# goroda/GPEXP

Hardware: AMD Instinct MI355X
Metric: GP-fit+IVAR-eval points/s at N=32768 d=8 (wall-time in ms_per_step); value = (N+M)/t_step, SURVEY 8d's N/t_fit and M/t_IVAR are points_per_s_fit / points_per_s_ivar right behind it (higher is better)
Workload: dtype f64; 1 GPU; C4: N=32768 d=8 Matern-5/2 (rho=0.5,s=1,noise=0.1) kfill+potrf+potrs+logdet+IVAR over M=32768 MC points; N=32768, d=8, M=32768, kernel=matern52, seed=32768, parallelism=1 GPU

## Files before the change

gpexp_amd/_lib.py:

```python
import ctypes as C
import os

import numpy as np

_HERE = os.path.dirname(os.path.abspath(__file__))
LIB_PATH = os.path.join(_HERE, "libgpx_hip.so")

c_i64 = C.c_int64
c_dp = C.POINTER(C.c_double)
c_ip = C.POINTER(c_i64)
c_vp = C.c_void_p

_SIGS = {
    "gpx_abi_version": (C.c_int, []),
    "gpx_last_error": (C.c_char_p, []),
    "gpx_create": (C.c_int, [C.c_int, C.POINTER(c_vp)]),
    "gpx_destroy": (C.c_int, [c_vp]),
    "gpx_sync": (C.c_int, [c_vp]),
    "gpx_trim": (C.c_int, [c_vp]),
    "gpx_device_info": (C.c_int, [c_vp, C.c_char_p, C.c_int, C.POINTER(C.c_int), c_ip, C.POINTER(C.c_int)]),
    "gpx_mat_from_host": (C.c_int, [c_vp, c_dp, c_i64, c_i64, C.c_int, C.POINTER(c_vp)]),
    "gpx_mat_alloc": (C.c_int, [c_vp, c_i64, c_i64, C.c_int, C.POINTER(c_vp)]),
    "gpx_mat_free": (C.c_int, [c_vp, c_vp]),
    "gpx_mat_clone": (C.c_int, [c_vp, c_vp, C.POINTER(c_vp)]),
# ... 149 lines not shown
    "gpx_program_capture": (C.c_int, [c_vp, c_ip, c_i64, c_ip, c_i64, C.POINTER(c_vp)]),
    "gpx_graph_launch": (C.c_int, [c_vp, c_vp, c_dp, c_ip]),
    "gpx_graph_free": (C.c_int, [c_vp, c_vp]),
    "gpx_dist2_unpack_rows": (C.c_int, [c_vp, c_vp, c_i64, c_i64, c_i64, c_i64, c_vp, c_i64, c_i64, c_i64]),
    "gpx_dist2_unpack_diag": (C.c_int, [c_vp, c_vp, c_i64, c_i64, c_i64, c_vp, c_i64]),
    "gpx_dist2_unpack_diag_at": (C.c_int, [c_vp, c_vp, c_i64, c_i64, c_i64, c_vp, c_i64, c_i64]),
    "gpx_dist2_trsv_diag": (C.c_int, [c_vp, c_vp, c_i64, c_i64, c_i64, c_vp, c_i64, C.c_int]),
    "gpx_dist2_gemv": (C.c_int, [c_vp, c_vp, c_i64, c_i64, c_i64, c_i64, c_vp, c_i64, c_vp, c_i64, C.c_int]),
    "gpx_dist2_logdet_acc": (C.c_int, [c_vp, c_vp, c_i64, c_i64, c_i64, c_i64, c_vp]),
    "gpx_stream_select": (C.c_int, [c_vp, C.c_int]),
    "gpx_event_record": (C.c_int, [c_vp, C.c_int]),
    "gpx_event_wait": (C.c_int, [c_vp, C.c_int]),
    "gpx_dist_finish": (C.c_int, [c_vp, c_vp]),
    "gpx_ivar_grad": (C.c_int, [c_vp, C.c_int, C.c_int, c_dp, C.c_int, c_vp, c_vp, c_vp, c_dp, c_dp]),
    "gpx_ivar_grad_w": (C.c_int, [c_vp, C.c_int, C.c_int, c_dp, C.c_int, c_vp, c_vp, c_vp, c_dp, c_vp, c_dp]),
    "gpx_ivar_grad_rows": (C.c_int, [c_vp, C.c_int, C.c_int, c_dp, C.c_int, c_vp, c_vp, c_vp, c_vp, c_i64, c_dp]),
    "gpx_var_grad": (C.c_int, [c_vp, C.c_int, C.c_int, c_dp, C.c_int, c_vp, c_vp, c_vp, c_dp, c_dp, c_dp, c_dp]),
    "gpx_var_grad_newpt": (C.c_int, [c_vp, C.c_int, C.c_int, c_dp, C.c_int, c_vp, c_vp, c_vp, c_dp]),
    "gpx_fitc_var_grad": (C.c_int, [c_vp, c_vp, C.c_int, C.c_int, c_dp, C.c_int, c_vp, c_vp, c_dp, c_dp, c_dp, c_dp]),
    "gpx_fitc_var_grad_newpt": (C.c_int, [c_vp, c_vp, C.c_int, C.c_int, c_dp, C.c_int, c_vp, c_vp, c_dp]),
    "gpx_vfe_design_create": (C.c_int, [c_vp, C.c_int, C.c_int, c_dp, C.c_int, c_vp, C.c_double, c_vp, C.POINTER(c_vp)]),
    "gpx_vfe_design_pin": (C.c_int, [c_vp, c_vp, c_vp]),
    "gpx_vfe_design_eval": (C.c_int, [c_vp, c_vp, c_vp, c_dp, c_dp]),
    "gpx_vfe_design_shape": (C.c_int, [c_vp, C.POINTER(c_i64), C.POINTER(c_i64), C.POINTER(c_i64)]),
    "gpx_vfe_design_free": (C.c_int, [c_vp, c_vp]),
    "gpx_vfe_var_grad": (C.c_int, [c_vp, c_vp, C.c_int, C.c_int, c_dp, C.c_int, c_vp, c_vp, c_vp, c_dp]),
    "gpx_vfe_var_grad_newpt": (C.c_int, [c_vp, c_vp, c_vp, c_vp, c_dp]),
    "gpx_profile_enable": (C.c_int, [c_vp, C.c_int]),
    "gpx_profile_reset": (C.c_int, [c_vp]),
    "gpx_profile_get": (C.c_int, [c_vp, C.c_int, c_ip, c_dp, c_dp, c_dp]),
    "gpx_dbg_gemm": (C.c_int, [c_vp, c_vp, c_vp, c_vp, C.c_int, C.c_int, C.c_int]),
    "gpx_dbg_gemm_strassen": (C.c_int, [c_vp, c_vp, c_vp, c_vp]),
    "gpx_dbg_gemm_strassen_depth": (C.c_int, [c_vp, c_vp, c_vp, c_vp, C.c_int]),
    "gpx_dbg_gemm_tri": (C.c_int, [c_vp, c_vp, c_vp, c_vp, C.c_int, C.c_int, C.c_int]),
    "gpx_dbg_gemm_ksplit": (C.c_int, [c_vp, c_vp, c_vp, c_vp, C.c_int, C.c_int]),
    "gpx_dbg_kfill_plan": (C.c_int, [c_vp, C.c_int, C.c_int, c_dp, C.c_int, c_vp, c_vp, C.POINTER(C.c_int), c_dp]),
    "gpx_dbg_colreduce_plan": (C.c_int, [c_i64, c_i64, C.POINTER(c_i64), C.POINTER(c_i64)]),
    "gpx_dbg_colreduce": (C.c_int, [c_vp, c_vp, c_i64, c_dp, c_dp, C.c_int]),
    "gpx_dbg_rowreduce": (C.c_int, [c_vp, c_vp, c_i64, c_dp, C.c_int, c_dp]),
    "gpx_dbg_sum": (C.c_int, [c_vp, c_dp, c_i64, c_dp]),
    "gpx_dbg_panel_bcast_plan": (C.c_int, [C.c_int, C.c_int, c_i64, C.c_int, C.POINTER(c_i64), C.POINTER(C.c_int),
                                           C.POINTER(c_i64), c_i64, C.POINTER(c_i64)]),
    "gpx_dbg_guard_violations": (c_i64, [c_vp]),
    "gpx_dbg_guard_selftest": (C.c_int, [c_vp]),
    "gpx_dbg_pool_stats": (C.c_int, [c_vp, C.POINTER(c_i64), C.POINTER(c_i64)]),
    "gpx_dbg_spin": (C.c_int, [c_vp, C.c_int]),
    "gpx_dbg_spin_us": (C.c_int, [c_vp, c_i64]),
    "gpx_dbg_stamp": (C.c_int, [c_vp, C.c_int]),
    "gpx_dbg_spin_until": (C.c_int, [c_vp, C.c_int, c_i64]),
    "gpx_dbg_event_elapsed": (C.c_int, [c_vp, C.c_int, C.c_int, c_dp]),
    "gpx_dbg_leaf_stamps": (C.c_int, [c_vp, c_vp, C.c_int, C.POINTER(c_i64)]),
    "gpx_dbg_greedy_var_scores": (C.c_int, [c_vp, C.c_int, C.c_int, c_dp, C.c_int, c_vp, c_ip, c_i64, c_dp]),
    "gpx_dbg_acq_epilogue": (C.c_int, [c_vp, C.c_int, C.c_double, c_dp, c_dp, c_i64, c_i64, c_dp, c_dp, C.POINTER(c_i64),
                                       c_dp]),
    "gpx_dbg_acq_mes_epilogue": (C.c_int, [c_vp, c_dp, c_i64, C.c_int, c_dp, c_dp, c_i64, c_i64, c_dp, c_dp, C.POINTER(c_i64), c_dp]),
}

_lib = None


def load():
    global _lib
    if _lib is not None:
        return _lib
    path = os.environ.get("GPX_LIB_PATH", LIB_PATH)
    if not os.path.exists(path):
# ... 49 lines not shown
```

gpexp_amd/csrc/api.hip:

```cpp
#include "gpx_internal.h"
#include <stdarg.h>
#include <stdio.h>
#include <string.h>
#include <math.h>
#include <stdlib.h>

static thread_local char g_err[1024] = "";

void gpx_set_error(const char* fmt, ...) {
  va_list ap;
  va_start(ap, fmt);
  vsnprintf(g_err, sizeof(g_err), fmt, ap);
  va_end(ap);
}

static constexpr int64_t GUARD = 4096;

int gpx_dev_alloc(gpx_ctx* ctx, int64_t bytes, void** out) {
  if (bytes <= 0) bytes = 8;
  bytes = gpx_round_up(bytes, 256);
  const int64_t key = bytes + (ctx->guard ? 2 * GUARD : 0);
  void* base = nullptr;
  auto it = ctx->pool.find(key);
  if (it != ctx->pool.end()) {
// ... 1318 lines not shown
                   : launch_gemm_ksplit_small(ctx, A->p, A->ld, B->p, B->ld, C->p, C->ld, m, n, k, mode == 3, parts, P);
}

int gpx_dbg_gemm(gpx_ctx* ctx, const gpx_mat* A, const gpx_mat* B, gpx_mat* C, int bt, int accumulate, int lower) {
  GPX_ARG(ctx && A && B && C, "NULL argument");
  const int64_t m = C->prows, n = C->pcols, k = A->pcols;
  GPX_ARG(A->prows == m, "A rows");
  GPX_ARG(bt ? (B->prows == n && B->pcols == k) : (B->prows == k && B->pcols == n), "B shape");
  GPX_TRY(launch_gemm(ctx, A->p, A->ld, B->p, B->ld, C->p, C->ld, m, n, k, bt != 0, accumulate != 0,
                      lower != 0));
  GPX_HIP(hipStreamSynchronize(ctx->stream));
  return 0;
}

int gpx_dbg_gemm_strassen(gpx_ctx* ctx, const gpx_mat* A, const gpx_mat* B, gpx_mat* C) {
  GPX_ARG(ctx && A && B && C, "NULL argument");
  const int64_t m = C->prows, n = C->pcols, k = A->pcols;
  GPX_ARG(A->prows == m && B->prows == k && B->pcols == n, "operand shapes");
  GPX_TRY(launch_gemm_strassen(ctx, A->p, A->ld, B->p, B->ld, C->p, C->ld, m, n, k, 1, nullptr, 0));
  GPX_HIP(hipStreamSynchronize(ctx->stream));
  return 0;
}

int gpx_dbg_gemm_strassen_depth(gpx_ctx* ctx, const gpx_mat* A, const gpx_mat* B, gpx_mat* C, int depth) {
  GPX_ARG(ctx && A && B && C, "NULL argument");
  GPX_ARG(depth >= 0 && depth <= GPX_STRASSEN_MAX_DEPTH, "strassen: depth out of range");
  const int64_t m = C->prows, n = C->pcols, k = A->pcols;
  GPX_ARG(A->prows == m && B->prows == k && B->pcols == n, "operand shapes");
  GPX_TRY(launch_gemm_strassen(ctx, A->p, A->ld, B->p, B->ld, C->p, C->ld, m, n, k, depth, nullptr, 0));
  GPX_HIP(hipStreamSynchronize(ctx->stream));
  return 0;
}

}
```

gpexp_amd/csrc/chol.hip:

```cpp
#include "gpx_internal.h"
#include <algorithm>
#include <math.h>
#include <stdlib.h>
#include <stddef.h>

namespace {

constexpr int NB = GPX_TILE;
constexpr int LS = NB + 1;

typedef double d4 __attribute__((ext_vector_type(4)));

__device__ __forceinline__ double readlane_d(double v, int srclane) {
  int lo = __builtin_amdgcn_readlane(__double2loint(v), srclane);
  int hi = __builtin_amdgcn_readlane(__double2hiint(v), srclane);
  return __hiloint2double(hi, lo);
}

constexpr int LB = 16;
constexpr int TS17 = LB + 1;
constexpr int BSZ = LB * TS17;
constexpr int LEAF_CB = LB * LB + 64 + LB;

__device__ __forceinline__ constexpr int sb_off(int I, int J) { return (I * (I + 1) / 2 + J) * BSZ; }
// ... 1208 lines not shown
    const int64_t o = blk_off(P, b0), sz = blk_off(P, b0 + 1) - o;
    hipLaunchKernelGGL(binv_gemv_kernel, dim3((unsigned)((sz + 3) / 4)), dim3(256), 0, ctx->stream, blk_inv(P, P.binvT, b0),
                       P.sib, sz, rhs + o, z + o, 0);
    return 0;
  }
  const int64_t mid = (b0 + b1) / 2;
  GPX_TRY(potrs_bwd(ctx, P, mid, b1, rhs, z));
  const int64_t r0 = blk_off(P, mid), r1 = blk_off(P, b1), c0 = blk_off(P, b0);
  GPX_TRY(launch_colreduce(ctx, P.L + r0 * P.ld + c0, P.ld, r1 - r0, r0 - c0, z + r0, rhs + c0, P.part, 1));
  return potrs_bwd(ctx, P, b0, mid, rhs, z);
}

#ifndef GPX_STRASSEN_MIN_ROWS
#define GPX_STRASSEN_MIN_ROWS 8192
#endif
#ifndef GPX_STRASSEN_MIN_COLS
#define GPX_STRASSEN_MIN_COLS 4096
#endif
#ifndef GPX_STRASSEN2_MIN_ROWS
#define GPX_STRASSEN2_MIN_ROWS 16384
#endif
#ifndef GPX_STRASSEN2_MIN_COLS
#define GPX_STRASSEN2_MIN_COLS 16384
#endif
static inline int strassen_gate(int64_t rows, int64_t cols, int64_t k) {
  if (!(rows >= GPX_STRASSEN_MIN_ROWS && k >= GPX_STRASSEN_MIN_ROWS && cols >= GPX_STRASSEN_MIN_COLS &&
        gemm_strassen_scratch_bytes(rows, cols, k, 1) > 0))
    return 0;
  if (!(rows >= GPX_STRASSEN2_MIN_ROWS && k >= GPX_STRASSEN2_MIN_ROWS && cols >= GPX_STRASSEN2_MIN_COLS &&
        gemm_strassen_scratch_bytes(rows, cols, k, 2) > 0))
    return 1;
  return 2;
}

static int trsm_left_oop_rec(gpx_ctx* ctx, const PotrsPlan& P, int64_t b0, int64_t b1, double* B, int64_t ldb, double* W,
                             int64_t ldw, int64_t m) {
  if (b1 - b0 == 1) {
    const int64_t o = blk_off(P, b0), sz = blk_off(P, b0 + 1) - o;
    return launch_gemm_tri(ctx, blk_inv(P, P.binv, b0), P.sib, B + o * ldb, ldb, W + o * ldw, ldw, sz, m, sz, false, false,
                           false, 1);
  }
  const int64_t mid = (b0 + b1) / 2;
  GPX_TRY(trsm_left_oop_rec(ctx, P, b0, mid, B, ldb, W, ldw, m));
  const int64_t r0 = blk_off(P, mid), r1 = blk_off(P, b1), c0 = blk_off(P, b0);
  const int depth = P.strassen ? std::min(P.strassen, strassen_gate(r1 - r0, m, r0 - c0)) : 0;
  if (depth > 0)
    GPX_TRY(launch_gemm_strassen(ctx, P.L + r0 * P.ld + c0, P.ld, W + c0 * ldw, ldw, B + r0 * ldb, ldb, r1 - r0, m, r0 - c0,
                                 depth, P.sscr, P.sscr_bytes));
  else
    GPX_TRY(launch_gemm(ctx, P.L + r0 * P.ld + c0, P.ld, W + c0 * ldw, ldw, B + r0 * ldb, ldb, r1 - r0, m, r0 - c0, false,
                        true, false));
  return trsm_left_oop_rec(ctx, P, mid, b1, B, ldb, W, ldw, m);
}

int chol_trsm_left_oop(gpx_ctx* ctx, gpx_mat* Lm, double* B, int64_t ldb, double* W, int64_t ldw, int64_t m) {
  GPX_ARG(Lm && Lm->factored && Lm->aux && B && W && B != W, "trsm: matrix has not been factored / bad buffers");
  if (m == 0) return 0;
  GPX_TRY(chol_binv_ensure(ctx, Lm));
  PotrsPlan P;
  P.L = Lm->p;
  P.ld = Lm->ld;
  P.n = Lm->prows;
  P.sib = Lm->binv_ib;
  P.ib = P.sib < 1024 ? P.sib : 1024;
  P.nblk = (P.n + P.ib - 1) / P.ib;
  P.binv = Lm->binv;
  P.binvT = nullptr;
  P.part = nullptr;
  void* ps = nullptr;
  int64_t sbytes = 0;
  int depth = 0;
  const int64_t max_depth = env_i64("GPX_STRASSEN", GPX_STRASSEN_MAX_DEPTH);
  if (P.nblk >= 2 && max_depth > 0) {
    const int64_t r0 = blk_off(P, P.nblk / 2);
    for (depth = (int)std::min<int64_t>(max_depth, strassen_gate(P.n - r0, m, r0)); depth > 0; --depth) {
      sbytes = gemm_strassen_scratch_bytes(P.n - r0, m, r0, depth);
      if (sbytes > 0 && gpx_dev_alloc(ctx, sbytes, &ps) == 0) break;
      (void)hipGetLastError();
// ... 105 lines not shown
```

gpexp_amd/csrc/gemm_f64.hip:

```cpp
#include "gpx_internal.h"
#include <stdlib.h>

namespace {

typedef double d4 __attribute__((ext_vector_type(4)));

constexpr int KB = 16;
constexpr int SA = KB + 1;

template <bool BT, int TE>
struct Smem {
  double a[2][TE * SA];
  double b[2][BT ? TE * SA : KB * (TE + 16)];
};

template <bool LOWER>
__device__ __forceinline__ bool tile_of(int sblk, int within, int tiles_m, int tiles_n, int sb_cols, int sb_shift,
                                        int* by, int* bx, int rot = 0) {
  const int sbm = (1 << sb_shift) - 1;
  int sr, sc;
  if (LOWER) {
    const int nsr = (tiles_m + sbm) >> sb_shift;
    const int noff = nsr * (nsr - 1) / 2;
    if (sblk < noff) {
// ... 397 lines not shown
  gemm_tile<false, true, TE, NoSeg, Multi>(sm, A, lda, B, ldb, dst.c[0], ldc, nk, by, bx, NoSeg(), dst);
}

template <bool BSIDE>
__global__ __launch_bounds__(256) void strassen_sums_kernel(const double* __restrict__ X, int64_t ldx, int64_t hr, int64_t hc,
                                                            double* __restrict__ S, int64_t lds, int64_t sstride) {
  const int64_t j = ((int64_t)blockIdx.x * 256 + threadIdx.x) * 2;
  if (j >= hc) return;
  for (int64_t i = blockIdx.y; i < hr; i += gridDim.y) {
    const double* x1 = X + i * ldx + j;
    const double* x2 = X + (i + hr) * ldx + j;
    const double2 x11 = *reinterpret_cast<const double2*>(x1);
    const double2 x12 = *reinterpret_cast<const double2*>(x1 + hc);
    const double2 x21 = *reinterpret_cast<const double2*>(x2);
    const double2 x22 = *reinterpret_cast<const double2*>(x2 + hc);
    double* o = S + i * lds + j;
#define GPX_S2(k_, ex_, ey_) *reinterpret_cast<double2*>(o + (k_) * sstride) = make_double2(ex_, ey_)
    GPX_S2(0, x11.x + x22.x, x11.y + x22.y);
    if (BSIDE) {
      GPX_S2(1, x12.x - x22.x, x12.y - x22.y);
      GPX_S2(2, x21.x - x11.x, x21.y - x11.y);
      GPX_S2(3, x11.x + x12.x, x11.y + x12.y);
      GPX_S2(4, x21.x + x22.x, x21.y + x22.y);
    } else {
      GPX_S2(1, x21.x + x22.x, x21.y + x22.y);
      GPX_S2(2, x11.x + x12.x, x11.y + x12.y);
      GPX_S2(3, x21.x - x11.x, x21.y - x11.y);
      GPX_S2(4, x12.x - x22.x, x12.y - x22.y);
    }
#undef GPX_S2
  }
}

template <bool BT, bool ACC>
__global__ __launch_bounds__(256, 2) void gemm_f64_batched_kernel(const double* A, int64_t lda, int64_t sa,
                                                                  const double* B, int64_t ldb, int64_t sb, double* C,
                                                                  int64_t ldc, int64_t sc, int nk, int tiles_n, int hiprio) {
  __shared__ Smem<BT, 64> sm;
  if (hiprio) __builtin_amdgcn_s_setprio(3);
  const int64_t b = blockIdx.y;
  const int by = blockIdx.x / tiles_n, bx = blockIdx.x - by * tiles_n;
  gemm_tile<BT, ACC, 64>(sm, A + b * sa, lda, B + b * sb, ldb, C + b * sc, ldc, nk, by, bx);
}

template <bool LOWER>
__global__ __launch_bounds__(256, 2) void gemm_f64_ksplit_kernel(const double* A, int64_t lda, const double* B, int64_t ldb,
                                                                 double* P, int64_t n, int64_t sp, int nk_slice, int parts,
                                                                 int tiles_m, int tiles_n, int sb_cols, int sb_shift) {
  __shared__ Smem<true, 128> sm;
  const int w = blockIdx.x, xcd = w & 7, q = w >> 3, sbs2 = 2 * sb_shift;
  const int job = (q >> sbs2) * 8 + xcd, within = q & ((1 << sbs2) - 1);
  int sb, slice;
  if (LOWER) {
    const int nsr = (tiles_m + (1 << sb_shift) - 1) >> sb_shift, noff = nsr * (nsr - 1) / 2;
    if (job < parts * noff) {
      slice = job / noff;
      sb = job - slice * noff;
    } else {
      const int jj = job - parts * noff;
      slice = jj / nsr;
      sb = noff + jj - slice * nsr;
    }
  } else {
    const int nsb = ((tiles_m + (1 << sb_shift) - 1) >> sb_shift) * sb_cols;
    slice = job / nsb;
    sb = job - slice * nsb;
// ... 278 lines not shown
  GPX_ARG(m % 128 == 0 && n % 128 == 0 && k % KB == 0 && k > 0 && m > 0 && n > 0, "gemm: m,n must be multiples of 128 and k of 16");
  GPX_ARG((lda % 2) == 0 && (ldb % 2) == 0, "gemm: leading dimensions must be even (16-byte loads)");
  GPX_ARG(dst.nd >= 1 && dst.nd <= GPX_MULTI_MAX, "gemm: bad destination count");
  const double tiles128 = (double)(m / 128) * (double)(n / 128);
  const int te = tiles128 < 1024.0 ? 64 : 128;
  const Plan p = make_plan(m, n, false, te);
  GPX_ARG(p.wgs < ((int64_t)1 << 31), "gemm: grid too large");
  const int nk = (int)(k / KB);
  ProfScope ps(ctx, GPX_PROF_GEMM, 2.0 * (double)m * (double)n * (double)k, 0.0);
  if (te == 64)
    hipLaunchKernelGGL(gemm_f64_multi_kernel<64>, dim3((unsigned)p.wgs), dim3(256), 0, ctx->stream, A, lda, B, ldb, dst, ldc, nk,
                       p.tm, p.tn, p.sbc, p.sb_shift);
  else
    hipLaunchKernelGGL(gemm_f64_multi_kernel<128>, dim3((unsigned)p.wgs), dim3(256), 0, ctx->stream, A, lda, B, ldb, dst, ldc, nk,
                       p.tm, p.tn, p.sbc, p.sb_shift);
  GPX_HIP(hipGetLastError());
  return 0;
}

static inline bool strassen_shape_ok(int64_t m, int64_t n, int64_t k, int depth) {
  return depth >= 1 && depth <= GPX_STRASSEN_MAX_DEPTH && m > 0 && n > 0 && k > 0 && m % ((int64_t)128 << depth) == 0 &&
         n % ((int64_t)128 << depth) == 0 && k % ((int64_t)KB << depth) == 0;
}

static inline int64_t strassen_level_elems(int64_t hm, int64_t hn, int64_t hk) {
  return 5 * (hm * gpx_skew_ld(hk) + hk * gpx_skew_ld(hn));
}

int64_t gemm_strassen_scratch_bytes(int64_t m, int64_t n, int64_t k, int depth) {
  if (!strassen_shape_ok(m, n, k, depth)) return 0;
  int64_t elems = 0;
  for (int d = 0; d < depth; ++d) {
    m /= 2, n /= 2, k /= 2;
    elems += strassen_level_elems(m, n, k);
  }
  return elems * 8;
}

namespace {
struct SDest {
  double* c;
  double s;
};
struct SProd {
  int a, b, nq, q[2];
  double s[2];
};
constexpr SProd kStrassen[7] = {
    {-1, -1, 2, {0, 3}, {1.0, 1.0}},
    {-2, 0, 2, {2, 3}, {1.0, -1.0}},
    {0, -2, 2, {1, 3}, {1.0, 1.0}},
    {3, -3, 2, {0, 2}, {1.0, 1.0}},
    {-3, 3, 2, {1, 0}, {1.0, -1.0}},
    {-4, -4, 1, {3, 0}, {1.0, 0.0}},
    {-5, -5, 1, {0, 0}, {1.0, 0.0}},
};
}

static int strassen_rec(gpx_ctx* ctx, const double* A, int64_t lda, const double* B, int64_t ldb, const SDest* dst, int nd,
                        int64_t ldc, int64_t m, int64_t n, int64_t k, int depth, double* scratch) {
  if (depth == 0) {
    for (int d = 1; d < nd; ++d)
      for (int e = 0; e < d; ++e) GPX_ARG(dst[d].c != dst[e].c, "strassen: two destinations of one product coincide");
    if (nd == 1 && dst[0].s == 1.0) return launch_gemm(ctx, A, lda, B, ldb, dst[0].c, ldc, m, n, k, false, true, false);
    if (nd == 2 && dst[0].s == 1.0) return launch_gemm_dual(ctx, A, lda, B, ldb, dst[0].c, dst[1].c, dst[1].s, ldc, m, n, k);
    GPX_ARG(nd >= 1 && nd <= GPX_MULTI_MAX, "strassen: too many destinations for one product");
    Multi md;
    for (int d = 0; d < GPX_MULTI_MAX; ++d) {
      md.c[d] = d < nd ? dst[d].c : nullptr;
      md.s[d] = d < nd ? dst[d].s : 0.0;
    }
    md.nd = nd;
    return launch_gemm_multi(ctx, A, lda, B, ldb, md, ldc, m, n, k);
  }
  const int64_t hm = m / 2, hn = n / 2, hk = k / 2, lsa = gpx_skew_ld(hk), lsb = gpx_skew_ld(hn);
  const int64_t sa = hm * lsa, sb = hk * lsb;
  double* const S = scratch;
  double* const T = scratch + 5 * sa;
  double* const below = T + 5 * sb;
  {
    ProfScope ps(ctx, GPX_PROF_REDUCE, 5.0 * (double)hm * hk + 5.0 * (double)hk * hn, 72.0 * ((double)hm * hk + (double)hk * hn));
    hipLaunchKernelGGL(strassen_sums_kernel<false>, dim3((unsigned)((hk / 2 + 255) / 256), (unsigned)(hm < 65535 ? hm : 65535)),
                       dim3(256), 0, ctx->stream, A, lda, hm, hk, S, lsa, sa);
    hipLaunchKernelGGL(strassen_sums_kernel<true>, dim3((unsigned)((hn / 2 + 255) / 256), (unsigned)(hk < 65535 ? hk : 65535)),
                       dim3(256), 0, ctx->stream, B, ldb, hk, hn, T, lsb, sb);
    if (hipGetLastError() != hipSuccess) {
      gpx_set_error("strassen: operand-sum launch failed");
      return -2;
    }
  }
  const int64_t qoff[4] = {0, hn, hm * ldc, hm * ldc + hn};
  for (const SProd& p : kStrassen) {
    const double* Ap = p.a < 0 ? S + (-1 - p.a) * sa : (p.a == 0 ? A : A + hm * lda + hk);
    const double* Bp = p.b < 0 ? T + (-1 - p.b) * sb : (p.b == 0 ? B : B + hk * ldb + hn);
    SDest sub[GPX_MULTI_MAX];
    int ns = 0;
    for (int d = 0; d < nd; ++d)
      for (int j = 0; j < p.nq; ++j) {
        GPX_ARG(ns < GPX_MULTI_MAX, "strassen: too many destinations for one product");
        sub[ns++] = SDest{dst[d].c + qoff[p.q[j]], dst[d].s * p.s[j]};
      }
    GPX_TRY(strassen_rec(ctx, Ap, p.a < 0 ? lsa : lda, Bp, p.b < 0 ? lsb : ldb, sub, ns, ldc, hm, hn, hk, depth - 1, below));
  }
  return 0;
}

int launch_gemm_strassen(gpx_ctx* ctx, const double* A, int64_t lda, const double* B, int64_t ldb, double* C, int64_t ldc,
                         int64_t m, int64_t n, int64_t k, int depth, double* scratch, int64_t scratch_bytes) {
  if (depth > GPX_STRASSEN_MAX_DEPTH) depth = GPX_STRASSEN_MAX_DEPTH;
  if ((lda % 2) != 0 || (ldb % 2) != 0 || C == A || C == B) depth = 0;
  void* own = nullptr;
  int64_t need = 0;
  for (; depth > 0; --depth) {
    need = gemm_strassen_scratch_bytes(m, n, k, depth);
    if (need == 0) continue;
    if (scratch && scratch_bytes >= need) break;
    if (gpx_dev_alloc(ctx, need, &own) == 0) {
      scratch = (double*)own;
      break;
    }
    (void)hipGetLastError();
    own = nullptr;
  }
  if (depth <= 0) return launch_gemm(ctx, A, lda, B, ldb, C, ldc, m, n, k, false, true, false);
  const SDest top{C, 1.0};
  const int r = strassen_rec(ctx, A, lda, B, ldb, &top, 1, ldc, m, n, k, depth, scratch);
  if (own) {
    (void)hipStreamSynchronize(ctx->stream);
    gpx_dev_release(ctx, own, need);
  }
  return r;
}

int launch_dist2_update(gpx_ctx* ctx, double* C, int64_t ldc, int64_t lr0, int64_t m, int64_t lc0, int64_t n, int64_t nb, int Pr,
                        int Pc, int pr, int pc, int64_t piece_stride, int64_t dsz, int nseg, const double* const* g,
                        const int64_t* ks, int below_diag) {
  if (m == 0 || n == 0 || nseg == 0) return 0;
  GPX_ARG(nseg > 0 && nseg <= GPX_SEG_MAX && Pr >= 1 && Pr <= GPX_MAX_PR && Pc >= 1, "dist2 update: too many segments / grid rows");
  GPX_ARG(m % 128 == 0 && n % 128 == 0 && nb % 128 == 0 && lr0 % nb == 0 && lc0 % nb == 0 && (ldc % 2) == 0, "dist2 update: alignment");
  Dist2Upd u;
  for (int s = 0; s < nseg; ++s) {
    u.g[s] = g[s];
    for (int p = 0; p < Pr; ++p) u.li0[s][p] = (int)(ks[s] + 1 <= p ? 0 : (ks[s] - p) / Pr + 1);
  }
  u.nseg = nseg;
  u.seg_nk = (int)(nb / KB);
  u.Pr = Pr; u.Pc = Pc; u.pr = pr; u.pc = pc;
  u.nb = (int)nb;
  u.gld = (int)gpx_g_ld(nb);
  u.li_first = (int)(lr0 / nb);
  u.lj_first = (int)(lc0 / nb);
  u.below_diag = below_diag;
  u.piece_stride = piece_stride;
  u.dsz = dsz;
  double tiles128 = 0.0;
  for (int64_t lj = lc0 / nb; lj * nb < lc0 + n; ++lj) {
    const int64_t J = lj * Pc + pc;
    const int64_t cw = (lc0 + n - lj * nb) < nb ? (lc0 + n - lj * nb) : nb;
    for (int64_t li = lr0 / nb; li * nb < lr0 + m; ++li) {
// ... 56 lines not shown
```

gpexp_amd/csrc/gpx_internal.h:

```cpp
#pragma once
#include <hip/hip_runtime.h>
#include <stdint.h>
#include <stdlib.h>
#include <string>
#include <vector>
#include <map>
#include <memory>
#include <unordered_set>
#include "../../include/gpx.h"
#include "../../include/gpx_dist.h"
#include "../../include/gpx_debug.h"

#define GPX_TILE 128
#define GPX_MAXD GPX_MAX_DIM
#define GPX_NSTREAMS 6
#define GPX_SEG_MAX 8
#ifndef GPX_G_SKEW
#define GPX_G_SKEW 0
#endif
#define GPX_MAX_PR 4

void gpx_set_error(const char* fmt, ...);
#define GPX_HIP(call)                                                                   \
  do {                                                                                  \
// ... 239 lines not shown
int gpx_posterior_chunk(gpx_ctx* ctx, const KParams& kp, const gpx_mat* L, const gpx_mat* X, const double* Zc, int64_t mc,
                        double* B, double* Wout, const double* alpha_dev, double* mean_dev, double* mean_host, double* ssq,
                        double* kd, double* part);
int posterior_cov_into(gpx_ctx* ctx, const KParams& kp, const gpx_mat* L, const gpx_mat* X, const gpx_mat* Z, Scratch& sc, double* C,
                       int64_t ldc);
int gpx_model_or_prior(const gpx_mat* L, const gpx_mat* X, const double* alpha, const char* msg, bool* prior);

int launch_kfill(gpx_ctx* ctx, const KParams& kp, const double* A, int64_t na, const double* B, int64_t nb,
                 int symmetric, const double* d_nugget, int64_t nugget_len, double nugget_scalar,
                 double* out, int64_t prows, int64_t pcols, int64_t ld);
int launch_kfill_offset(gpx_ctx* ctx, const KParams& kp, const double* X, int64_t n, int64_t row_off, int64_t col_off,
                        const double* d_nugget, int64_t nugget_len, double nugget_scalar, double* out, int64_t prows,
                        int64_t pcols, int64_t ld);
int launch_kdiag(gpx_ctx* ctx, const KParams& kp, const double* Z, int64_t m, double* out);
int launch_kfill_cyclic(gpx_ctx* ctx, const KParams& kp, const double* X, int64_t n, const double* d_nugget,
                        int64_t nugget_len, double nugget_scalar, double* out, int64_t prows, int64_t pcols, int64_t ld,
                        int64_t nb, int Pr, int pr, int Pc, int pc);
int gpx_copy2d(gpx_ctx* ctx, const double* src, int64_t lds_, double* dst, int64_t ldd, int64_t rows, int64_t cols);
int gpx_copy2d_lower(gpx_ctx* ctx, const double* src, int64_t lds_, double* dst, int64_t ldd, int64_t n);
int launch_kfill_rows(gpx_ctx* ctx, const KParams& kp, const double* X, int64_t n, int64_t row0, const double* d_nugget,
                      int64_t nugget_len, double nugget_scalar, double* out, int64_t prows_band, int64_t pcols,
                      int64_t ld);

static inline int gpx_chain_prio(const gpx_ctx* ctx) { return ctx->stream == ctx->streams[1] ? 1 : 0; }
int launch_gemm(gpx_ctx* ctx, const double* A, int64_t lda, const double* B, int64_t ldb, double* C, int64_t ldc,
                int64_t m, int64_t n, int64_t k, bool bt, bool accumulate, bool lower);

int launch_gemm_tri(gpx_ctx* ctx, const double* A, int64_t lda, const double* B, int64_t ldb, double* C, int64_t ldc,
                    int64_t m, int64_t n, int64_t k, bool bt, bool accumulate, bool lower, int tri);
constexpr int GPX_STRASSEN_MAX_DEPTH = 2;
int64_t gemm_strassen_scratch_bytes(int64_t m, int64_t n, int64_t k, int depth);
int launch_gemm_strassen(gpx_ctx* ctx, const double* A, int64_t lda, const double* B, int64_t ldb, double* C, int64_t ldc,
                         int64_t m, int64_t n, int64_t k, int depth, double* scratch, int64_t scratch_bytes);
int launch_gemm_ksplit(gpx_ctx* ctx, const double* A, int64_t lda, const double* B, int64_t ldb, double* C, int64_t ldc,
                       int64_t m, int64_t n, int64_t k, bool lower, int64_t parts, double* P, bool assign = false);
int launch_gemm_ksplit_small(gpx_ctx* ctx, const double* A, int64_t lda, const double* B, int64_t ldb, double* C, int64_t ldc,
                             int64_t m, int64_t n, int64_t k, bool assign, int64_t parts, double* P);
int launch_gemm_batched(gpx_ctx* ctx, const double* A, int64_t lda, int64_t sa, const double* B, int64_t ldb, int64_t sb,
                        double* C, int64_t ldc, int64_t sc, int64_t m, int64_t n, int64_t k, bool bt, bool accumulate,
                        int64_t batch);

int launch_dist2_update(gpx_ctx* ctx, double* C, int64_t ldc, int64_t lr0, int64_t m, int64_t lc0, int64_t n, int64_t nb, int Pr,
                        int Pc, int pr, int pc, int64_t piece_stride, int64_t dsz, int nseg, const double* const* g,
                        const int64_t* ks, int below_diag);

int launch_leaf(gpx_ctx* ctx, double* A, int64_t ld, double* inv, int64_t base_index, int64_t n_valid);
int chol_potrf(gpx_ctx* ctx, double* A, int64_t ld, int64_t n, double* invd, int64_t n_valid);
int chol_potrf_nozero(gpx_ctx* ctx, double* A, int64_t ld, int64_t n, double* invd, int64_t base, int64_t n_valid);
int chol_trsm_right(gpx_ctx* ctx, const double* L, int64_t ldl, const double* invd, double* X, int64_t ldx,
                    int64_t m, int64_t n);
int chol_trsm_right_n(gpx_ctx* ctx, const double* L, int64_t ldl, const double* invd, double* X, int64_t ldx,
                      int64_t m, int64_t n);
int chol_trsm_left(gpx_ctx* ctx, const double* L, int64_t ldl, const double* invd, double* B, int64_t ldb,
                   int64_t n, int64_t m);
int chol_trsv(gpx_ctx* ctx, const double* L, int64_t ld, const double* invd, double* y, int64_t n, bool transposed);
int64_t chol_trsv_scratch_bytes(int64_t n);
int chol_trsv_with_scratch(gpx_ctx* ctx, const double* L, int64_t ld, const double* invd, double* y, int64_t n,
                           bool transposed, double* scratch);
int launch_logdet(gpx_ctx* ctx, const double* L, int64_t ld, int64_t n, double* d_out);
int chol_trtri(gpx_ctx* ctx, const gpx_mat* L, double* Linv, double* tmp);
int chol_binv_ensure(gpx_ctx* ctx, gpx_mat* L);
int chol_trsm_right_trailing(gpx_ctx* ctx, gpx_mat* L, int64_t r0, double* X, int64_t ldx, int64_t m, int transposed, double* T);
int chol_trsm_right_leading(gpx_ctx* ctx, gpx_mat* L, int64_t ncols, double* X, int64_t ldx, int64_t m, double* T, int64_t tcap);
int chol_trsm_right_n_leading(gpx_ctx* ctx, gpx_mat* L, int64_t ncols, double* X, int64_t ldx, int64_t m, double* T);
int chol_block_inverse(gpx_ctx* ctx, const double* D, int64_t ldd, const double* invd, double* inv, int64_t w, double* tmp);
int64_t chol_binv_order(int64_t n);
// ... 137 lines not shown
```

gpexp_amd/device.py:

```python
import ctypes as C
import atexit
import os

import numpy as np

from . import _lib
from ._lib import check, as_f64, dptr, c_vp, c_i64, GpxError

K_SE, K_MATERN32, K_MATERN52, K_MEHLER = 0, 1, 2, 3
PROF_CLASSES = ["kfill", "gemm", "leaf", "trsv", "reduce", "greedy", "comm", "kcross"]

_ctx = None


class Context:

    def __init__(self, device=None):
        self.lib = _lib.load()
        if device is None:
            device = int(os.environ.get("LOCAL_RANK", "0"))
        h = c_vp()
        rc = self.lib.gpx_create(int(device), C.byref(h))
        if rc != 0:
            raise RuntimeError("gpexp_amd needs an MI355X: " + self.lib.gpx_last_error().decode())
# ... 1135 lines not shown


def var_grad_newpt(ctx, spec, L, X, Z):
    out = np.empty(Z.shape[0] * spec.d)
    check(ctx.lib.gpx_var_grad_newpt(ctx.h, *spec.args(), L.h, X.h, Z.h, dptr(out)))
    return out


def kfill_plan(ctx, spec, X, Z=None):
    ex = C.c_int()
    cen = np.zeros(spec.d)
    check(ctx.lib.gpx_dbg_kfill_plan(ctx.h, *spec.args(), X.h, Z.h if Z is not None else None, C.byref(ex), dptr(cen)))
    return bool(ex.value), cen


def dbg_gemm_tri(ctx, A, B, Cm, bt, accumulate, tri):
    check(ctx.lib.gpx_dbg_gemm_tri(ctx.h, A.h, B.h, Cm.h, int(bt), int(accumulate), int(tri)))


def dbg_gemm_ksplit(ctx, A, B, Cm, mode, parts):
    check(ctx.lib.gpx_dbg_gemm_ksplit(ctx.h, A.h, B.h, Cm.h, int(mode), int(parts)))


def dbg_gemm(ctx, A, B, Cm, bt, accumulate, lower=False):
    check(ctx.lib.gpx_dbg_gemm(ctx.h, A.h, B.h, Cm.h, int(bt), int(accumulate), int(lower)))


def dbg_gemm_strassen(ctx, A, B, Cm):
    check(ctx.lib.gpx_dbg_gemm_strassen(ctx.h, A.h, B.h, Cm.h))


def dbg_gemm_strassen_depth(ctx, A, B, Cm, depth):
    check(ctx.lib.gpx_dbg_gemm_strassen_depth(ctx.h, A.h, B.h, Cm.h, int(depth)))
```

include/gpx_debug.h:

```cpp
#ifndef GPX_DEBUG_H
#define GPX_DEBUG_H
#include "gpx.h"
#ifdef __cplusplus
extern "C" {
#endif

int gpx_dbg_gemm(gpx_ctx* ctx, const gpx_mat* A, const gpx_mat* B, gpx_mat* C, int bt, int accumulate, int lower);
int gpx_dbg_gemm_tri(gpx_ctx* ctx, const gpx_mat* A, const gpx_mat* B, gpx_mat* C, int bt, int accumulate, int tri);
int gpx_dbg_gemm_ksplit(gpx_ctx* ctx, const gpx_mat* A, const gpx_mat* B, gpx_mat* C, int mode, int parts);
int gpx_dbg_gemm_strassen(gpx_ctx* ctx, const gpx_mat* A, const gpx_mat* B, gpx_mat* C);
int gpx_dbg_gemm_strassen_depth(gpx_ctx* ctx, const gpx_mat* A, const gpx_mat* B, gpx_mat* C, int depth);
int gpx_dbg_spin(gpx_ctx* ctx, int ms);
int64_t gpx_dbg_guard_violations(gpx_ctx* ctx);
int gpx_dbg_pool_stats(gpx_ctx* ctx, int64_t* pooled_bytes, int64_t* outstanding_bytes);
int gpx_dbg_guard_selftest(gpx_ctx* ctx);
int gpx_dbg_panel_bcast_plan(int W, int me, int64_t small_elems, int npieces, const int64_t* counts, const int* roots,
                             int64_t* ops, int64_t max_ops, int64_t* nops);
int gpx_dbg_colreduce_plan(int64_t rows, int64_t pcols, int64_t* nchunk, int64_t* bound_elems);
int gpx_dbg_colreduce(gpx_ctx* ctx, const gpx_mat* B, int64_t rows, const double* v, double* out, int subtract);
int gpx_dbg_rowreduce(gpx_ctx* ctx, const gpx_mat* A, int64_t cols, const double* v, int weighted_squares, double* out);
int gpx_dbg_sum(gpx_ctx* ctx, const double* x, int64_t n, double* out);
int gpx_dbg_kfill_plan(gpx_ctx* ctx, int kind, int d, const double* hyp, int nhyp, const gpx_mat* X, const gpx_mat* Z,
                       int* exact, double* center);

int gpx_dbg_spin_us(gpx_ctx* ctx, int64_t us);
int gpx_dbg_stamp(gpx_ctx* ctx, int slot);
int gpx_dbg_spin_until(gpx_ctx* ctx, int slot, int64_t us);
int gpx_dbg_event_elapsed(gpx_ctx* ctx, int id0, int id1, double* ms);

int gpx_dbg_leaf_stamps(gpx_ctx* ctx, gpx_mat* K, int fast, int64_t* out30);

int gpx_dbg_greedy_var_scores(gpx_ctx* ctx, int kind, int d, const double* hyp, int nhyp, const gpx_mat* C, const int64_t* keep,
                              int64_t nkeep, double* out_d );

int gpx_dbg_qei_blocks(gpx_ctx* ctx, int kind, int d, const double* hyp, int nhyp, const gpx_mat* L, const gpx_mat* X,
                       const double* alpha, const gpx_mat* Zb, int64_t q, double nugget, double* mean, double* Cb, double* Fb);

int gpx_dbg_vfe_qei_blocks(gpx_ctx* ctx, const gpx_fitc* f, const gpx_mat* S, const double* coeff, const gpx_mat* Zb, int64_t q,
                           double nugget, double* mean, double* Cb, double* Fb);

int gpx_dbg_acq_epilogue(gpx_ctx* ctx, int acq, double param, const double* mean, const double* var, int64_t m, int64_t chunk,
                         double* cost, double* coef , int64_t* best, double* best_cost);

int gpx_dbg_acq_mes_epilogue(gpx_ctx* ctx, const double* ystar, int64_t K, int sign, const double* mean, const double* var, int64_t m,
// ... 7 lines not shown
```

Before: 104,600 points/s.

## Fuse two Strassen levels of operand sums and extend Strassen to more solve GEMMs

Adds a kernel that forms both levels of Strassen operand sums (first-level S/T plus all seven second-level sum sets) in one pass over each quadrant, instead of launching sum kernels at every recursion level. This removes repeated reads of the operands and many small launches at the second level. The cost is scratch that grows sevenfold at the deepest level and a heavy register footprint in the new kernel. A new gate3 also enables depth-1 Strassen for triangular-solve GEMM updates with at least 4096 rows and 32768 columns when the solve already uses depth 2. That widens the use of the faster but less accurate Strassen path in potrs.

Result: no change. 105,300 points/s (median of 6 runs) (+0.7%).

```diff
diff --git a/gpexp_amd/_lib.py b/gpexp_amd/_lib.py
--- a/gpexp_amd/_lib.py
+++ b/gpexp_amd/_lib.py
@@ -205,6 +205,8 @@
     "gpx_dbg_gemm": (C.c_int, [c_vp, c_vp, c_vp, c_vp, C.c_int, C.c_int, C.c_int]),
     "gpx_dbg_gemm_strassen": (C.c_int, [c_vp, c_vp, c_vp, c_vp]),
     "gpx_dbg_gemm_strassen_depth": (C.c_int, [c_vp, c_vp, c_vp, c_vp, C.c_int]),
+    "gpx_dbg_gemm_strassen_sums": (C.c_int, [c_vp, c_vp, c_vp, c_vp, C.c_int, C.c_int]),
+    "gpx_dbg_strassen_gate3": (C.c_int, [c_i64, c_i64, c_i64, c_i64, c_i64, c_i64]),
     "gpx_dbg_gemm_tri": (C.c_int, [c_vp, c_vp, c_vp, c_vp, C.c_int, C.c_int, C.c_int]),
     "gpx_dbg_gemm_ksplit": (C.c_int, [c_vp, c_vp, c_vp, c_vp, C.c_int, C.c_int]),
     "gpx_dbg_kfill_plan": (C.c_int, [c_vp, C.c_int, C.c_int, c_dp, C.c_int, c_vp, c_vp, C.POINTER(C.c_int), c_dp]),
diff --git a/gpexp_amd/csrc/api.hip b/gpexp_amd/csrc/api.hip
--- a/gpexp_amd/csrc/api.hip
+++ b/gpexp_amd/csrc/api.hip
@@ -1374,4 +1374,32 @@
   return 0;
 }
 
-}
+int gpx_dbg_gemm_strassen_sums(gpx_ctx* ctx, const gpx_mat* A, const gpx_mat* B, gpx_mat* C, int depth, int fused) {
+  GPX_ARG(ctx && A && B && C, "NULL argument");
+  GPX_ARG(depth >= 0 && depth <= GPX_STRASSEN_MAX_DEPTH, "strassen: depth out of range");
+  const int64_t m = C->prows, n = C->pcols, k = A->pcols;
+  GPX_ARG(A->prows == m && B->prows == k && B->pcols == n, "operand shapes");
+  constexpr int64_t band = 32;
+  constexpr double sentinel = -7.25;
+  int64_t need = 0;
+  for (int d = depth; d > 0 && need == 0; --d) need = gemm_strassen_scratch_bytes(m, n, k, d);
+  Scratch sc(ctx);
+  double* s;
+  GPX_TRY(sc.get(need + band * 8, &s));
+  double h[band];
+  std::fill(h, h + band, sentinel);
+  GPX_HIP(hipMemcpyAsync(s + need / 8, h, sizeof h, hipMemcpyHostToDevice, ctx->stream));
+  GPX_HIP(hipStreamSynchronize(ctx->stream));
+  GPX_TRY(launch_gemm_strassen_sums(ctx, A->p, A->ld, B->p, B->ld, C->p, C->ld, m, n, k, depth, s, need, fused != 0));
+  std::fill(h, h + band, 0.0);
+  GPX_HIP(hipMemcpyAsync(h, s + need / 8, sizeof h, hipMemcpyDeviceToHost, ctx->stream));
+  GPX_HIP(hipStreamSynchronize(ctx->stream));
+  for (int64_t i = 0; i < band; ++i) GPX_ARG(h[i] == sentinel, "strassen: an operand-sum launch wrote behind the last sum of its scratch");
+  return 0;
+}
+
+int gpx_dbg_strassen_gate3(int64_t rows, int64_t cols, int64_t k, int64_t top_rows, int64_t top_cols, int64_t top_k) {
+  return chol_strassen_gate3(rows, cols, k, chol_strassen_gate(top_rows, top_cols, top_k));
+}
+
+}
diff --git a/gpexp_amd/csrc/chol.hip b/gpexp_amd/csrc/chol.hip
--- a/gpexp_amd/csrc/chol.hip
+++ b/gpexp_amd/csrc/chol.hip
@@ -1264,6 +1264,18 @@
     return 1;
   return 2;
 }
+int chol_strassen_gate(int64_t rows, int64_t cols, int64_t k) { return strassen_gate(rows, cols, k); }
+
+#ifndef GPX_STRASSEN3_MIN_ROWS
+#define GPX_STRASSEN3_MIN_ROWS 4096
+#endif
+#ifndef GPX_STRASSEN3_MIN_COLS
+#define GPX_STRASSEN3_MIN_COLS 32768
+#endif
+int chol_strassen_gate3(int64_t rows, int64_t cols, int64_t k, int solve_depth) {
+  return solve_depth >= 2 && rows >= GPX_STRASSEN3_MIN_ROWS && k >= GPX_STRASSEN3_MIN_ROWS && cols >= GPX_STRASSEN3_MIN_COLS &&
+         gemm_strassen_scratch_bytes(rows, cols, k, 1) > 0;
+}
 
 static int trsm_left_oop_rec(gpx_ctx* ctx, const PotrsPlan& P, int64_t b0, int64_t b1, double* B, int64_t ldb, double* W,
                              int64_t ldw, int64_t m) {
@@ -1275,7 +1287,8 @@
   const int64_t mid = (b0 + b1) / 2;
   GPX_TRY(trsm_left_oop_rec(ctx, P, b0, mid, B, ldb, W, ldw, m));
   const int64_t r0 = blk_off(P, mid), r1 = blk_off(P, b1), c0 = blk_off(P, b0);
-  const int depth = P.strassen ? std::min(P.strassen, strassen_gate(r1 - r0, m, r0 - c0)) : 0;
+  int depth = P.strassen ? std::min(P.strassen, strassen_gate(r1 - r0, m, r0 - c0)) : 0;
+  if (depth == 0 && chol_strassen_gate3(r1 - r0, m, r0 - c0, P.strassen)) depth = 1;
   if (depth > 0)
     GPX_TRY(launch_gemm_strassen(ctx, P.L + r0 * P.ld + c0, P.ld, W + c0 * ldw, ldw, B + r0 * ldb, ldb, r1 - r0, m, r0 - c0,
                                  depth, P.sscr, P.sscr_bytes));
diff --git a/gpexp_amd/csrc/gemm_f64.hip b/gpexp_amd/csrc/gemm_f64.hip
--- a/gpexp_amd/csrc/gemm_f64.hip
+++ b/gpexp_amd/csrc/gemm_f64.hip
@@ -453,6 +453,68 @@
   }
 }
 
+template <bool BSIDE>
+__device__ __forceinline__ void strassen_five(const double2 (&y)[4], double2 (&s)[5]) {
+#define GPX_ADD(a_, b_) make_double2((a_).x + (b_).x, (a_).y + (b_).y)
+#define GPX_SUB(a_, b_) make_double2((a_).x - (b_).x, (a_).y - (b_).y)
+  s[0] = GPX_ADD(y[0], y[3]);
+  if (BSIDE) {
+    s[1] = GPX_SUB(y[1], y[3]);
+    s[2] = GPX_SUB(y[2], y[0]);
+    s[3] = GPX_ADD(y[0], y[1]);
+    s[4] = GPX_ADD(y[2], y[3]);
+  } else {
+    s[1] = GPX_ADD(y[2], y[3]);
+    s[2] = GPX_ADD(y[0], y[1]);
+    s[3] = GPX_SUB(y[2], y[0]);
+    s[4] = GPX_SUB(y[1], y[3]);
+  }
+#undef GPX_ADD
+#undef GPX_SUB
+}
+
+template <bool BSIDE>
+__global__ __launch_bounds__(256) void strassen_sums2_kernel(const double* __restrict__ X, int64_t ldx, int64_t qr, int64_t qc,
+                                                             double* __restrict__ S, int64_t lds, int64_t sstride,
+                                                             double* __restrict__ S2, int64_t lds2, int64_t sstride2,
+                                                             int64_t pstride2) {
+  const int64_t j = ((int64_t)blockIdx.x * 256 + threadIdx.x) * 2;
+  if (j >= qc) return;
+  for (int64_t i = blockIdx.y; i < qr; i += gridDim.y) {
+    double2 x[4][4];
+#pragma unroll
+    for (int a = 0; a < 4; ++a)
+#pragma unroll
+      for (int b = 0; b < 4; ++b)
+        x[a][b] = *reinterpret_cast<const double2*>(X + ((a >> 1) * 2 * qr + (b >> 1) * qr + i) * ldx + (a & 1) * 2 * qc +
+                                                    (b & 1) * qc + j);
+    double2 s1[5][4];
+#pragma unroll
+    for (int b = 0; b < 4; ++b) {
+      const double2 y[4] = {x[0][b], x[1][b], x[2][b], x[3][b]};
+      double2 s[5];
+      strassen_five<BSIDE>(y, s);
+      double* o = S + ((b >> 1) * qr + i) * lds + (b & 1) * qc + j;
+#pragma unroll
+      for (int k = 0; k < 5; ++k) {
+        s1[k][b] = s[k];
+        *reinterpret_cast<double2*>(o + k * sstride) = s[k];
+      }
+    }
+    double* o2 = S2 + i * lds2 + j;
+#pragma unroll
+    for (int p = 0; p < 7; ++p) {
+      const int src = BSIDE ? (p == 0 ? 0 : p == 1 ? -1 : p == 2 ? 1 : p == 3 ? 2 : p == 4 ? -4 : p - 2)
+                            : (p == 0 ? 0 : p == 1 ? 1 : p == 2 ? -1 : p == 3 ? -4 : p - 2);
+      const double2(&q)[4] = src >= 0 ? s1[src] : x[-1 - src];
+      double2 s[5];
+      strassen_five<BSIDE>(q, s);
+#pragma unroll
+      for (int k = 0; k < 5; ++k) *reinterpret_cast<double2*>(o2 + p * pstride2 + k * sstride2) = s[k];
+    }
+  }
+}
+
 template <bool BT, bool ACC>
 __global__ __launch_bounds__(256, 2) void gemm_f64_batched_kernel(const double* A, int64_t lda, int64_t sa,
                                                                   const double* B, int64_t ldb, int64_t sb, double* C,
@@ -797,7 +859,7 @@
   int64_t elems = 0;
   for (int d = 0; d < depth; ++d) {
     m /= 2, n /= 2, k /= 2;
-    elems += strassen_level_elems(m, n, k);
+    elems += (depth >= 2 && d == depth - 1 ? 7 : 1) * strassen_level_elems(m, n, k);
   }
   return elems * 8;
 }
@@ -822,8 +884,14 @@
 };
 }
 
+enum SSums {
+  SSUMS_LEVEL = 0,
+  SSUMS_PAIR = 1,
+  SSUMS_FORMED = 2,
+};
+
 static int strassen_rec(gpx_ctx* ctx, const double* A, int64_t lda, const double* B, int64_t ldb, const SDest* dst, int nd,
-                        int64_t ldc, int64_t m, int64_t n, int64_t k, int depth, double* scratch) {
+                        int64_t ldc, int64_t m, int64_t n, int64_t k, int depth, double* scratch, SSums sums) {
   if (depth == 0) {
     for (int d = 1; d < nd; ++d)
       for (int e = 0; e < d; ++e) GPX_ARG(dst[d].c != dst[e].c, "strassen: two destinations of one product coincide");
@@ -843,7 +911,22 @@
   double* const S = scratch;
   double* const T = scratch + 5 * sa;
   double* const below = T + 5 * sb;
-  {
+  const bool pair = sums == SSUMS_PAIR && depth == 2;
+  int64_t below_stride = 0;
+  if (pair) {
+    const int64_t qm = hm / 2, qn = hn / 2, qk = hk / 2, lsa2 = gpx_skew_ld(qk), lsb2 = gpx_skew_ld(qn);
+    const int64_t sa2 = qm * lsa2, sb2 = qk * lsb2;
+    below_stride = strassen_level_elems(qm, qn, qk);
+    ProfScope ps(ctx, GPX_PROF_REDUCE, 13.75 * ((double)hm * hk + (double)hk * hn), 142.0 * ((double)hm * hk + (double)hk * hn));
+    hipLaunchKernelGGL(strassen_sums2_kernel<false>, dim3((unsigned)((qk / 2 + 255) / 256), (unsigned)(qm < 65535 ? qm : 65535)),
+                       dim3(256), 0, ctx->stream, A, lda, qm, qk, S, lsa, sa, below, lsa2, sa2, below_stride);
+    hipLaunchKernelGGL(strassen_sums2_kernel<true>, dim3((unsigned)((qn / 2 + 255) / 256), (unsigned)(qk < 65535 ? qk : 65535)),
+                       dim3(256), 0, ctx->stream, B, ldb, qk, qn, T, lsb, sb, below + 5 * sa2, lsb2, sb2, below_stride);
+    if (hipGetLastError() != hipSuccess) {
+      gpx_set_error("strassen: operand-sum launch failed");
+      return -2;
+    }
+  } else if (sums != SSUMS_FORMED) {
     ProfScope ps(ctx, GPX_PROF_REDUCE, 5.0 * (double)hm * hk + 5.0 * (double)hk * hn, 72.0 * ((double)hm * hk + (double)hk * hn));
     hipLaunchKernelGGL(strassen_sums_kernel<false>, dim3((unsigned)((hk / 2 + 255) / 256), (unsigned)(hm < 65535 ? hm : 65535)),
                        dim3(256), 0, ctx->stream, A, lda, hm, hk, S, lsa, sa);
@@ -855,7 +938,8 @@
     }
   }
   const int64_t qoff[4] = {0, hn, hm * ldc, hm * ldc + hn};
-  for (const SProd& p : kStrassen) {
+  for (int pi = 0; pi < 7; ++pi) {
+    const SProd& p = kStrassen[pi];
     const double* Ap = p.a < 0 ? S + (-1 - p.a) * sa : (p.a == 0 ? A : A + hm * lda + hk);
     const double* Bp = p.b < 0 ? T + (-1 - p.b) * sb : (p.b == 0 ? B : B + hk * ldb + hn);
     SDest sub[GPX_MULTI_MAX];
@@ -865,13 +949,20 @@
         GPX_ARG(ns < GPX_MULTI_MAX, "strassen: too many destinations for one product");
         sub[ns++] = SDest{dst[d].c + qoff[p.q[j]], dst[d].s * p.s[j]};
       }
-    GPX_TRY(strassen_rec(ctx, Ap, p.a < 0 ? lsa : lda, Bp, p.b < 0 ? lsb : ldb, sub, ns, ldc, hm, hn, hk, depth - 1, below));
+    GPX_TRY(strassen_rec(ctx, Ap, p.a < 0 ? lsa : lda, Bp, p.b < 0 ? lsb : ldb, sub, ns, ldc, hm, hn, hk, depth - 1,
+                         below + pi * below_stride, pair ? SSUMS_FORMED : sums));
   }
   return 0;
 }
 
 int launch_gemm_strassen(gpx_ctx* ctx, const double* A, int64_t lda, const double* B, int64_t ldb, double* C, int64_t ldc,
                          int64_t m, int64_t n, int64_t k, int depth, double* scratch, int64_t scratch_bytes) {
+  return launch_gemm_strassen_sums(ctx, A, lda, B, ldb, C, ldc, m, n, k, depth, scratch, scratch_bytes, true);
+}
+
+int launch_gemm_strassen_sums(gpx_ctx* ctx, const double* A, int64_t lda, const double* B, int64_t ldb, double* C, int64_t ldc,
+                              int64_t m, int64_t n, int64_t k, int depth, double* scratch, int64_t scratch_bytes,
+                              bool pair_sums) {
   if (depth > GPX_STRASSEN_MAX_DEPTH) depth = GPX_STRASSEN_MAX_DEPTH;
   if ((lda % 2) != 0 || (ldb % 2) != 0 || C == A || C == B) depth = 0;
   void* own = nullptr;
@@ -889,7 +980,7 @@
   }
   if (depth <= 0) return launch_gemm(ctx, A, lda, B, ldb, C, ldc, m, n, k, false, true, false);
   const SDest top{C, 1.0};
-  const int r = strassen_rec(ctx, A, lda, B, ldb, &top, 1, ldc, m, n, k, depth, scratch);
+  const int r = strassen_rec(ctx, A, lda, B, ldb, &top, 1, ldc, m, n, k, depth, scratch, pair_sums ? SSUMS_PAIR : SSUMS_LEVEL);
   if (own) {
     (void)hipStreamSynchronize(ctx->stream);
     gpx_dev_release(ctx, own, need);
diff --git a/gpexp_amd/csrc/gpx_internal.h b/gpexp_amd/csrc/gpx_internal.h
--- a/gpexp_amd/csrc/gpx_internal.h
+++ b/gpexp_amd/csrc/gpx_internal.h
@@ -295,6 +295,10 @@
 int64_t gemm_strassen_scratch_bytes(int64_t m, int64_t n, int64_t k, int depth);
 int launch_gemm_strassen(gpx_ctx* ctx, const double* A, int64_t lda, const double* B, int64_t ldb, double* C, int64_t ldc,
                          int64_t m, int64_t n, int64_t k, int depth, double* scratch, int64_t scratch_bytes);
+int launch_gemm_strassen_sums(gpx_ctx* ctx, const double* A, int64_t lda, const double* B, int64_t ldb, double* C, int64_t ldc,
+                              int64_t m, int64_t n, int64_t k, int depth, double* scratch, int64_t scratch_bytes, bool pair_sums);
+int chol_strassen_gate(int64_t rows, int64_t cols, int64_t k);
+int chol_strassen_gate3(int64_t rows, int64_t cols, int64_t k, int solve_depth);
 int launch_gemm_ksplit(gpx_ctx* ctx, const double* A, int64_t lda, const double* B, int64_t ldb, double* C, int64_t ldc,
                        int64_t m, int64_t n, int64_t k, bool lower, int64_t parts, double* P, bool assign = false);
 int launch_gemm_ksplit_small(gpx_ctx* ctx, const double* A, int64_t lda, const double* B, int64_t ldb, double* C, int64_t ldc,
diff --git a/gpexp_amd/device.py b/gpexp_amd/device.py
--- a/gpexp_amd/device.py
+++ b/gpexp_amd/device.py
@@ -1191,3 +1191,11 @@
 
 def dbg_gemm_strassen_depth(ctx, A, B, Cm, depth):
     check(ctx.lib.gpx_dbg_gemm_strassen_depth(ctx.h, A.h, B.h, Cm.h, int(depth)))
+
+
+def dbg_gemm_strassen_sums(ctx, A, B, Cm, depth, fused):
+    check(ctx.lib.gpx_dbg_gemm_strassen_sums(ctx.h, A.h, B.h, Cm.h, int(depth), int(bool(fused))))
+
+
+def dbg_strassen_gate3(rows, cols, k, top_rows, top_cols, top_k):
+    return int(_lib.load().gpx_dbg_strassen_gate3(int(rows), int(cols), int(k), int(top_rows), int(top_cols), int(top_k)))
diff --git a/include/gpx_debug.h b/include/gpx_debug.h
--- a/include/gpx_debug.h
+++ b/include/gpx_debug.h
@@ -10,6 +10,8 @@
 int gpx_dbg_gemm_ksplit(gpx_ctx* ctx, const gpx_mat* A, const gpx_mat* B, gpx_mat* C, int mode, int parts);
 int gpx_dbg_gemm_strassen(gpx_ctx* ctx, const gpx_mat* A, const gpx_mat* B, gpx_mat* C);
 int gpx_dbg_gemm_strassen_depth(gpx_ctx* ctx, const gpx_mat* A, const gpx_mat* B, gpx_mat* C, int depth);
+int gpx_dbg_gemm_strassen_sums(gpx_ctx* ctx, const gpx_mat* A, const gpx_mat* B, gpx_mat* C, int depth, int fused);
+int gpx_dbg_strassen_gate3(int64_t rows, int64_t cols, int64_t k, int64_t top_rows, int64_t top_cols, int64_t top_k);
 int gpx_dbg_spin(gpx_ctx* ctx, int ms);
 int64_t gpx_dbg_guard_violations(gpx_ctx* ctx);
 int gpx_dbg_pool_stats(gpx_ctx* ctx, int64_t* pooled_bytes, int64_t* outstanding_bytes);
diff --git a/profiles/strassen_sums2_isa_compare.py b/profiles/strassen_sums2_isa_compare.py
--- /dev/null
+++ b/profiles/strassen_sums2_isa_compare.py
@@ -0,0 +1,51 @@
+#!/usr/bin/env python3
+import os
+import re
+import sys
+
+sys.path.insert(0, os.path.dirname(os.path.abspath(__file__)))
+from strassen2_isa_compare import functions
+
+KEYS = ("vgpr_count", "agpr_count", "sgpr_count", "vgpr_spill_count", "sgpr_spill_count", "private_segment_fixed_size",
+        "group_segment_fixed_size")
+
+
+def kernel_metadata(path):
+    out, cur = {}, {}
+    for line in open(path):
+        m = re.match(r"^\s+(?:- )?\.(\w+):\s+(\S+)\s*$", line)
+        if not m:
+            continue
+        key, val = m.group(1), m.group(2)
+        if key in KEYS:
+            cur[key] = int(val)
+        elif key == "name":
+            cur["name"] = val
+        elif key == "wavefront_size":
+            if "name" in cur:
+                out[cur["name"]] = cur
+            cur = {}
+    return out
+
+
+def main():
+    parent, change = sys.argv[1], sys.argv[2]
+    bad = 0
+    for f in ("gemm_f64.s", "chol.s"):
+        a, b = functions(os.path.join(parent, f)), functions(os.path.join(change, f))
+        diff = [n for n in sorted(a) if n not in b or a[n] != b[n]]
+        for n in diff:
+            print("%s: %s %s" % (f, "MISSING  " if n not in b else "DIFFERENT", n))
+        bad += len(diff)
+        print("%s: %d functions in the parent, %d identical in the change, %d new: %s"
+              % (f, len(a), len(a) - len(diff), len(set(b) - set(a)), " ".join(sorted(set(b) - set(a)))))
+    for name, md in sorted(kernel_metadata(os.path.join(change, "gemm_f64.s")).items()):
+        if "strassen_sums" not in name:
+            continue
+        print("%s: %s" % (name, "  ".join("%s=%d" % (k, md[k]) for k in KEYS if k in md)))
+        bad += md.get("vgpr_spill_count", 0) + md.get("sgpr_spill_count", 0) + md.get("private_segment_fixed_size", 0) > 0
+    return 1 if bad else 0
+
+
+if __name__ == "__main__":
+    sys.exit(main())
```
